# dsshim0125/s2p

Hardware: AMD Instinct MI355X
Metric: G+D train-step images/sec at 84x84 bs=64/GPU (higher is better)
Workload: dtype bf16; 1 GPU; configs[2]: full G+D train step (hinge GAN + feature matching + VGG19 perceptual + L1, Adam x2), 84x84 cheetah, netG=s2p, netD=multiscale(2); global_batch=64, per_gpu_batch=64, parallelism=dp1, hip_graph=True, graph_segments=1, streams=overlapped, vgg_weights=seeded stand-in (ImageNet weights unobtainable offline)

## Files before the change

### include/s2p_hip.h

```cpp
#ifndef S2P_HIP_H
#define S2P_HIP_H
#include <stddef.h>
#include <stdint.h>

#ifdef __cplusplus
extern "C" {
#endif
#pragma GCC visibility push(default)

#define S2P_VERSION 125

enum { S2P_F32 = 0, S2P_BF16 = 1 };
enum { S2P_ACT_NONE = 0, S2P_ACT_RELU = 1, S2P_ACT_LRELU = 2, S2P_ACT_TANH = 3, S2P_ACT_SWISH = 4 };
enum { S2P_EPI_STORE = 0,
       S2P_EPI_ADD = 1,
       S2P_EPI_MUL_ACTGRAD = 2   };

typedef struct {
  int32_t dtype;
  int32_t N, H, W, Cin, x_pitch;
  int32_t Ho, Wo, Cout, y_pitch;
  int32_t KH, KW, stride, pad;
  int32_t transposed;
  int32_t reflect;
// ... 24 lines not shown
                       size_t workspace_bytes, void* stream);
int s2p_conv2d_dgrad_mat(const s2p_conv_desc* d, const void* dy, const void* w_bwd, void* d_mid, const void* aux, const void* xn,
                         int xn_pitch, const float* stats, const void* gb_img, int gb_pitch, const float* gb_st,
                         int gb_st_pitch, int act, float slope, float eps, float* sums, void* dxn, int dxn_pitch,
                         void* dgb_img, int dgb_pitch, float* dgb_st, int dgb_st_pitch, const void* res, int res_pitch,
                         void* workspace, size_t workspace_bytes, void* stream);
int s2p_conv2d_mat_is_fused(const s2p_conv_desc* d, int dgrad, int has_gb);
enum { S2P_CONV_PATH_THIN = 0, S2P_CONV_PATH_THIN4 = 1, S2P_CONV_PATH_THIN_CIN = 2, S2P_CONV_PATH_THIN_ROWS = 3,
       S2P_CONV_PATH_PLANE = 4, S2P_CONV_PATH_PLANEG = 5, S2P_CONV_PATH_HALO = 6, S2P_CONV_PATH_SPLITK = 7,
       S2P_CONV_PATH_DMA = 8, S2P_CONV_PATH_PHASES = 9, S2P_CONV_PATH_GENERIC = 10 };
enum { S2P_HALO_S9_176_PIPE = 0, S2P_HALO_S9_176 = 1, S2P_HALO_S9_320 = 2, S2P_HALO_R_176 = 3, S2P_HALO_R_320 = 4 };
int s2p_conv2d_path(const s2p_conv_desc* d, int dgrad, int has_workspace);
int s2p_conv2d_wgrad(const s2p_conv_desc* d, const void* x, const void* dy, float* dw, float* db,
                     int cin_real, int cout_real, int64_t dw_gstride, int splitk, void* stream);
size_t s2p_conv2d_wgrad_workspace(const s2p_conv_desc* d, int cin_real, int cout_real);
int s2p_conv2d_wgrad_ws(const s2p_conv_desc* d, const void* x, const void* dy, float* dw, float* db,
                        int cin_real, int cout_real, int64_t dw_gstride, int splitk, void* workspace,
                        size_t workspace_bytes, void* stream);
size_t s2p_conv2d_wgrad_det_workspace(const s2p_conv_desc* d, int cin_real, int cout_real, int splitk);
typedef struct { const void* x; const void* dy; float* dw; float* db; } s2p_wgrad_job;
size_t s2p_conv2d_wgrad_batched_workspace(const s2p_conv_desc* d, int n_jobs, int cin_real, int cout_real);
int s2p_conv2d_wgrad_batched(const s2p_conv_desc* d, const s2p_wgrad_job* jobs, int n_jobs, int cin_real,
                             int cout_real, void* workspace, size_t workspace_bytes, void* stream);
int s2p_reflect_pad_bwd(int dtype, const void* dxp, int N, int H, int W, int C, int pad, void* dx,
                        void* stream);
int s2p_channel_sum(int dtype, const void* dy, int64_t pixels, int C, int pitch, float* db,
                    void* stream);
size_t s2p_channel_sum_workspace(int64_t pixels, int C);
int s2p_channel_sum_ws(int dtype, const void* dy, int64_t pixels, int C, int pitch, float* db, void* workspace,
                       size_t workspace_bytes, void* stream);

int64_t s2p_in_stats_floats(int N, int HW, int C);
int s2p_in_stats(int dtype, const void* x, int N, int HW, int C, int pitch, float eps,
                 float* stats, void* stream);
int s2p_in_apply_fwd(int dtype, const void* x, int N, int HW, int C, int pitch,
                     const float* stats, const void* gb_img, int gb_pitch,
                     const float* gb_st, int gb_st_pitch, int act, float slope, float eps,
                     void* y, int y_pitch, void* stream);
int s2p_in_norm_fwd(int dtype, const void* x, int N, int HW, int C, int pitch, const void* gb_img, int gb_pitch,
                    const float* gb_st, int gb_st_pitch, int act, float slope, float eps, void* y, int y_pitch,
                    float* stats, void* stream);
int64_t s2p_in_bwd_sums_floats(int N, int HW, int C);
int s2p_in_bwd_reduce(int dtype, const void* da, int da_pitch, const void* x, int N, int HW, int C,
                      int pitch, const float* stats, const void* gb_img, int gb_pitch,
                      const float* gb_st, int gb_st_pitch, int act, float slope, float eps,
                      float* sums, void* stream);
// ... 184 lines not shown
```

### s2p_amd/_lib.py

```python
import ctypes
import os
import subprocess

import torch

_HERE = os.path.dirname(os.path.abspath(__file__))
_SO = os.path.join(_HERE, "csrc", "libs2p_hip.so")

F32, BF16 = 0, 1
ACT_NONE, ACT_RELU, ACT_LRELU, ACT_TANH, ACT_SWISH = 0, 1, 2, 3, 4
EPI_STORE, EPI_ADD, EPI_MUL_ACTGRAD = 0, 1, 2
(PATH_THIN, PATH_THIN4, PATH_THIN_CIN, PATH_THIN_ROWS, PATH_PLANE, PATH_PLANEG, PATH_HALO, PATH_SPLITK, PATH_DMA, PATH_PHASES,
 PATH_GENERIC) = range(11)
HALO_S9_176_PIPE, HALO_S9_176, HALO_S9_320, HALO_R_176, HALO_R_320 = range(5)

c_int, c_float, c_void_p, c_int64 = ctypes.c_int, ctypes.c_float, ctypes.c_void_p, ctypes.c_int64


class ConvDesc(ctypes.Structure):
    _fields_ = [(n, ctypes.c_int32) for n in (
        "dtype", "N", "H", "W", "Cin", "x_pitch", "Ho", "Wo", "Cout", "y_pitch",
        "KH", "KW", "stride", "pad", "transposed", "reflect", "groups", "x_gstride", "y_gstride", "cin_real")]


# ... 34 lines not shown
SIGNATURES = {
    "s2p_version": [],
    "s2p_last_error": [],
    "s2p_conv2d_fwd": [_DESC, _P, _P, _P, _P, _P, c_int, c_float, c_int, _P],
    "s2p_conv2d_dgrad": [_DESC, _P, _P, _P, _P, _P, c_int, c_int, c_float, _P],
    "s2p_conv2d_fwd_workspace": [_DESC, c_int],
    "s2p_conv2d_fwd_ws": [_DESC, _P, _P, _P, _P, _P, c_int, c_float, c_int, _P, ctypes.c_size_t, _P],
    "s2p_conv2d_fwd_mat": [_DESC, _P, _P, _P, _P, _P, c_int, _P, c_int, _P, c_int, c_int, c_float, c_float, _P, c_int, _P, _P,
                           ctypes.c_size_t, _P],
    "s2p_conv2d_dgrad_mat": [_DESC, _P, _P, _P, _P, _P, c_int, _P, _P, c_int, _P, c_int, c_int, c_float, c_float, _P, _P, c_int, _P, c_int,
                             _P, c_int, _P, c_int, _P, ctypes.c_size_t, _P],
    "s2p_conv2d_mat_is_fused": [_DESC, c_int, c_int],
    "s2p_conv2d_path": [_DESC, c_int, c_int],
    "s2p_conv2d_dgrad_workspace": [_DESC],
    "s2p_conv2d_dgrad_ws": [_DESC, _P, _P, _P, _P, _P, c_int, c_int, c_float, _P, ctypes.c_size_t, _P],
    "s2p_conv2d_wgrad": [_DESC, _P, _P, _P, _P, c_int, c_int, c_int64, c_int, _P],
    "s2p_conv2d_wgrad_workspace": [_DESC, c_int, c_int],
    "s2p_conv2d_wgrad_det_workspace": [_DESC, c_int, c_int, c_int],
    "s2p_channel_sum_workspace": [c_int64, c_int],
    "s2p_channel_sum_ws": [c_int, _P, c_int64, c_int, c_int, _P, _P, ctypes.c_size_t, _P],
    "s2p_conv2d_wgrad_ws": [_DESC, _P, _P, _P, _P, c_int, c_int, c_int64, c_int, _P, ctypes.c_size_t, _P],
    "s2p_conv2d_wgrad_batched_workspace": [_DESC, c_int, c_int, c_int],
    "s2p_conv2d_wgrad_batched": [_DESC, ctypes.POINTER(WgradJob), c_int, c_int, c_int, _P, ctypes.c_size_t, _P],
    "s2p_reflect_pad_bwd": [c_int, _P, c_int, c_int, c_int, c_int, c_int, _P, _P],
    "s2p_channel_sum": [c_int, _P, c_int64, c_int, c_int, _P, _P],
    "s2p_in_stats": [c_int, _P, c_int, c_int, c_int, c_int, c_float, _P, _P],
    "s2p_in_apply_fwd": [c_int, _P, c_int, c_int, c_int, c_int, _P, _P, c_int, _P, c_int, c_int, c_float,
                         c_float, _P, c_int, _P],
    "s2p_in_norm_fwd": [c_int, _P, c_int, c_int, c_int, c_int, _P, c_int, _P, c_int, c_int, c_float, c_float, _P, c_int,
                        _P, _P],
    "s2p_in_bwd_reduce": [c_int, _P, c_int, _P, c_int, c_int, c_int, c_int, _P, _P, c_int, _P, c_int, c_int,
                          c_float, c_float, _P, _P],
    "s2p_in_bwd_apply": [c_int, _P, c_int, _P, c_int, c_int, c_int, c_int, _P, _P, c_int, _P, c_int, c_int,
                         c_float, c_float, _P, _P, c_int, _P, c_int, _P, c_int, _P],
    "s2p_in_norm_bwd": [c_int, _P, c_int, _P, c_int, c_int, c_int, c_int, _P, _P, c_int, _P, c_int, c_int,
                        c_float, c_float, _P, _P, c_int, _P, c_int, _P, c_int, _P],
    "s2p_in_norm_bwd_res": [c_int, _P, c_int, _P, c_int, c_int, c_int, c_int, _P, _P, c_int, _P, c_int, c_int,
                            c_float, c_float, _P, _P, c_int, _P, c_int, _P, c_int, _P, c_int, _P],
    "s2p_in_stats_floats": [c_int, c_int, c_int],
    "s2p_in_bwd_sums_floats": [c_int, c_int, c_int],
    "s2p_linear_fwd": [_P, c_int, c_int, c_int, _P, c_int, _P, c_int, c_int, c_float, _P, c_int, c_int, _P],
    "s2p_linear_bwd_workspace": [c_int, c_int, c_int],
    "s2p_linear_bwd": [_P, c_int, _P, c_int, _P, c_int, c_int, c_int, c_int, c_int, _P, c_int, c_int, c_float, _P, c_int, _P, _P,
                       c_int, _P, ctypes.c_size_t, _P],
    "s2p_gauss_head_fwd": [_P, c_int, c_int, c_int, _P, c_int, _P, c_int, _P, c_int, _P, c_int, _P, c_int, _P],
    "s2p_gauss_head_bwd": [_P, c_int, c_int, c_int, _P, c_int, _P, c_int, _P, c_int, _P, c_int, _P, c_int, _P, c_int, _P],
# ... 130 lines not shown
```

### s2p_amd/csrc/wgrad_slab.hip

```cpp
#include "wgrad_slab_core.h"

constexpr int WS_MAX_JOBS = 16;
struct WgSlabArgs {
  const void* A[WS_MAX_JOBS]; const void* B[WS_MAX_JOBS]; float* dW[WS_MAX_JOBS]; float* db[WS_MAX_JOBS];
  float* slab; float* slabb;
  WgsRaster g;
  int Cin;
  int co_tiles, tiles_per_job;
  int S, blocks_per_split, nblocks;
  int halo;
  int toff[9];
  int total_wgs;
};

template <int WROWS, bool TBL>
__global__ __launch_bounds__(256, 2) void wgrad_slab_kernel(const WgSlabArgs a) {
  constexpr int T = 9, NXI = WROWS / 32;
  constexpr int TOFF = TBL ? WGS_TBL_BYTES : 0;
  __shared__ __attribute__((aligned(1024))) char lds_all[TOFF + WGS_NST * wgs_stage_bytes(NXI)];
  const int f = wgs_xcd_spread(blockIdx.x, a.total_wgs);
  const int per_job = a.tiles_per_job * a.S;
  const int job = f / per_job;
  const int rem = f - job * per_job;
  const int split = rem / a.tiles_per_job, tile = rem - split * a.tiles_per_job;
  const int co_t = tile % a.co_tiles, ci_s = tile / a.co_tiles;
  const int b0 = split * a.blocks_per_split;
  int b1 = b0 + a.blocks_per_split; if (b1 > a.nblocks) b1 = a.nblocks;
  const int nblk = b1 - b0;
  const int wave = __builtin_amdgcn_readfirstlane(threadIdx.x >> 6);
  const bool do_bias = a.db[job] != nullptr && ci_s == 0 && (wave & 1) == 0;
  const WgsRaster g = {a.g.N, a.g.Ha, a.g.Wa, a.g.Ha, a.g.Wa, a.g.Hp, a.g.Wp, 1, 0, 0, a.g.a_pitch, a.g.b_pitch, a.g.a_bytes, a.g.b_bytes};

  f32x16 acc[T];
  f32x16 accb;
  wgs_accumulate<T, NXI, TBL>(g, a.A[job], a.B[job], a.toff, a.halo, co_t, ci_s, b0, nblk, do_bias, lds_all + TOFF,
                              (unsigned*)lds_all, acc, accb);

  const int tile_g = job * a.tiles_per_job + tile;
  if (a.S == 1) {
    const int lane = threadIdx.x & 63, r = lane & 31, h = lane >> 5, wa = wave >> 1, wb = wave & 1;
    float* dW = a.dW[job];
    const int row_len = T * a.Cin;
#pragma unroll
    for (int t = 0; t < T; ++t)
#pragma unroll
      for (int e = 0; e < 16; ++e) {
        const int co = co_t * 64 + 32 * wa + (e & 3) + 8 * (e >> 2) + 4 * h;
        float* o = dW + (size_t)co * row_len + t * a.Cin + ci_s * 64 + 32 * wb + r;
        *o += acc[t][e];
      }
    if (do_bias && r == 0) {
      float* db = a.db[job];
#pragma unroll
      for (int e = 0; e < 16; ++e) db[co_t * 64 + 32 * wa + (e & 3) + 8 * (e >> 2) + 4 * h] += accb[e];
    }
  } else {
    wgs_store_slab<T>(a.slab + ((size_t)tile_g * a.S + split) * (64 * T * 64), a.slabb + ((size_t)tile_g * a.S + split) * 64, acc, accb, do_bias);
  }
}

__global__ __launch_bounds__(256) void wgrad_slab_reduce_kernel(const WgSlabArgs a) {
  constexpr int T = 9;
  const int tile_g = blockIdx.x / T, t = blockIdx.x - tile_g * T;
  const int job = tile_g / a.tiles_per_job, tile = tile_g - job * a.tiles_per_job;
  const int co_t = tile % a.co_tiles, ci_s = tile / a.co_tiles;
  const float* sl = a.slab + (size_t)tile_g * a.S * (64 * T * 64);
  float* dW = a.dW[job];
  const int row_len = T * a.Cin;
#pragma unroll
  for (int u = 0; u < 4; ++u) {
    const int i = threadIdx.x + 256 * u;
    const int qd = i & 15, row = i >> 4;
    const size_t so = ((size_t)(row * T + t) * 16 + qd) * 4;
    f32x4 s = *(const f32x4*)(sl + so);
    for (int k = 1; k < a.S; ++k) s += *(const f32x4*)(sl + (size_t)k * (64 * T * 64) + so);
    float* o = dW + (size_t)(co_t * 64 + row) * row_len + t * a.Cin + ci_s * 64 + qd * 4;
    *(f32x4*)o = *(const f32x4*)o + s;
  }
  if (t == 0 && a.db[job] != nullptr && ci_s == 0 && threadIdx.x < 64) {
    const float* sb = a.slabb + (size_t)tile_g * a.S * 64;
    float s = sb[threadIdx.x];
    for (int k = 1; k < a.S; ++k) s += sb[k * 64 + threadIdx.x];
// ... 72 lines not shown
  bool tbl;
  a.g = ws_raster(d); wgs_limits(a.g, tbl);
  const int Wp = a.g.Wp;
  a.Cin = d->Cin;
  a.co_tiles = d->Cout / 64; a.tiles_per_job = a.co_tiles * (d->Cin / 64);
  a.nblocks = cdiv((long long)d->N * a.g.Hp * Wp, 64);
  a.S = ws_splits(d, n_jobs);
  a.blocks_per_split = cdiv(a.nblocks, a.S);
  a.halo = Wp + 1;
  const int wrows = ws_window_rows(a.halo);
  for (int ky = 0; ky < 3; ++ky)
    for (int kx = 0; kx < 3; ++kx) a.toff[ky * 3 + kx] = (ky - 1) * Wp + (kx - 1);
  const int tiles = n_jobs * a.tiles_per_job;
  a.total_wgs = tiles * a.S;
  if (a.S > 1) {
    const size_t need = (size_t)tiles * a.S * (64 * 9 * 64 + 64) * sizeof(float);
    if (!workspace || workspace_bytes < need)
      S2P_FAIL(-1, "s2p_conv2d_wgrad_batched: workspace of %zu bytes needed (s2p_conv2d_wgrad_batched_workspace), got %zu", need, workspace_bytes);
    a.slab = (float*)workspace;
    a.slabb = a.slab + (size_t)tiles * a.S * (64 * 9 * 64);
  }
  hipStream_t st = (hipStream_t)stream;
  dim3 grid(a.total_wgs);
  if (wrows <= 128) { if (tbl) hipLaunchKernelGGL((wgrad_slab_kernel<128, true>), grid, dim3(256), 0, st, a); else hipLaunchKernelGGL((wgrad_slab_kernel<128, false>), grid, dim3(256), 0, st, a); }
  else if (wrows <= 192) { if (tbl) hipLaunchKernelGGL((wgrad_slab_kernel<192, true>), grid, dim3(256), 0, st, a); else hipLaunchKernelGGL((wgrad_slab_kernel<192, false>), grid, dim3(256), 0, st, a); }
  else { if (tbl) hipLaunchKernelGGL((wgrad_slab_kernel<256, true>), grid, dim3(256), 0, st, a); else hipLaunchKernelGGL((wgrad_slab_kernel<256, false>), grid, dim3(256), 0, st, a); }
  S2P_CHECK_LAUNCH("wgrad_slab_kernel");
  if (a.S > 1) {
    hipLaunchKernelGGL(wgrad_slab_reduce_kernel, dim3(tiles * 9), dim3(256), 0, st, a);
    S2P_CHECK_LAUNCH("wgrad_slab_reduce_kernel");
  }
  return 0;
}
```

### s2p_amd/csrc/wgrad_slab_core.h

```cpp
#pragma once
#include "s2p_common.h"

struct WgsRaster {
  int N, Ha, Wa, Hb, Wb, Hp, Wp, bs, py, px;
  int a_pitch, b_pitch;
  unsigned a_bytes, b_bytes;
};

constexpr int WGS_TBL_MAX = 768;
constexpr int WGS_TBL_BYTES = 2 * WGS_TBL_MAX * 4;
constexpr int WGS_NST = 3;
constexpr int wgs_stage_bytes(int nxi) { return (64 + nxi * 32) * 128; }

__device__ __forceinline__ int wgs_xcd_spread(int bid, int nw) {
  const int q8 = nw >> 3, r8 = nw & 7, xcd = bid & 7, k = bid >> 3;
  return (xcd < r8 ? xcd * (q8 + 1) : r8 * (q8 + 1) + (xcd - r8) * q8) + k;
}

template <int T, int NXI, bool TBL>
__device__ __forceinline__ void wgs_accumulate(const WgsRaster& g, const void* A, const void* B, const int* toff, const int halo,
                                               const int co_t, const int ci_s, const int b0, const int nblk, const bool do_bias,
                                               char* const smem, unsigned* const ptab, f32x16 (&acc)[T], f32x16& accb) {
  constexpr int RS = 128, NST = WGS_NST;
  constexpr int ASTG = 64 * RS;
  constexpr int STG = wgs_stage_bytes(NXI);
  constexpr int NDMA = 2 + NXI;
  const int tid = threadIdx.x, lane = tid & 63;
  const int wave = __builtin_amdgcn_readfirstlane(tid >> 6);

  const unsigned OOB = 0x80000000u;
  const i32x4 ar = s2p_make_rsrc(A, g.a_bytes);
  const i32x4 br = s2p_make_rsrc(B, g.b_bytes);
  const unsigned lds0 = __builtin_amdgcn_readfirstlane(s2p_lds_addr(smem));

  const int lrow = lane >> 3, pch = lane & 7;
  const int a_cbyte = (co_t * 64) * 2, b_cbyte = (ci_s * 64) * 2;
  int pn[NDMA], prr[NDMA], pc[NDMA];
  int cb[NDMA];
  unsigned q4[NDMA], noffc[NDMA], tv[NDMA];
  const int HpWp = g.Hp * g.Wp;
  if constexpr (TBL) {
    for (int q = tid; q < HpWp; q += 256) {
      const int r = q / g.Wp, c = q - r * g.Wp;
      ptab[q] = (c < g.Wa && r < g.Ha) ? (unsigned)(r * g.Wa + c) * (unsigned)(g.a_pitch * 2) : 0xc0000000u;
      const int sy = r * g.bs + g.py, sx = c * g.bs + g.px;
      ptab[WGS_TBL_MAX + q] = (sy < g.Hb && sx < g.Wb) ? (unsigned)(sy * g.Wb + sx) * (unsigned)(g.b_pitch * 2) : 0xc0000000u;
    }
    __syncthreads();
  }
#pragma unroll
  for (int i = 0; i < NDMA; ++i) {
    const int row = (4 * (i < 2 ? i : i - 2) + wave) * 8 + lrow;
    int pos = b0 * 64 + row - (i < 2 ? 0 : halo);
    int nadj = 0;
    if (pos < 0) { pos += g.Hp * g.Wp; nadj = -1; }
    cb[i] = (i < 2 ? a_cbyte : b_cbyte) + ((pch ^ (((row >> 1) & 1) << 2)) * 16);
    if constexpr (TBL) {
      const int n = pos / HpWp, q = pos - n * HpWp;
      q4[i] = (unsigned)q * 4u;
      noffc[i] = (unsigned)((n + nadj) * (i < 2 ? g.Ha * g.Wa * g.a_pitch * 2 : g.Hb * g.Wb * g.b_pitch * 2) + cb[i]);
      tv[i] = ptab[(i < 2 ? 0 : WGS_TBL_MAX) + q];
    } else {
      const int q1 = pos / g.Wp;
      pc[i] = pos - q1 * g.Wp;
      const int n = q1 / g.Hp;
      prr[i] = q1 - n * g.Hp;
      pn[i] = n + nadj;
    }
  }
  const int a_pitch2 = g.a_pitch * 2, b_pitch2 = g.b_pitch * 2;
  const int adv_q = 64 / g.Wp, adv_c = 64 - adv_q * g.Wp, adv_n = adv_q / g.Hp, adv_r = adv_q - adv_n * g.Hp;
  const int tadv_n = 64 / HpWp;
  const unsigned tadv_q4 = (unsigned)(64 - tadv_n * HpWp) * 4u, HpWp4 = (unsigned)HpWp * 4u;
  const unsigned img_a = (unsigned)(g.Ha * g.Wa) * (unsigned)a_pitch2, img_b = (unsigned)(g.Hb * g.Wb) * (unsigned)b_pitch2;
  auto issue_one = [&](auto ic, unsigned base) {
    constexpr int i = decltype(ic)::value;
    if constexpr (TBL) {
      const unsigned off = tv[i] + noffc[i];
      if (i < 2) s2p_dma16(ar, base + (4 * i + wave) * 1024, (int)off);
      else s2p_dma16(br, base + ASTG + (4 * (i - 2) + wave) * 1024, (int)off);
      const unsigned img = i < 2 ? img_a : img_b;
      const unsigned qa = q4[i] + tadv_q4;
      const bool wrap = qa >= HpWp4;
      q4[i] = wrap ? qa - HpWp4 : qa;
      noffc[i] += (unsigned)tadv_n * img + (wrap ? img : 0u);
      tv[i] = *(const unsigned*)((const char*)(ptab + (i < 2 ? 0 : WGS_TBL_MAX)) + q4[i]);
    } else {
      int off;
      if constexpr (i < 2) {
        const bool ok = pc[i] < g.Wa && prr[i] < g.Ha && (unsigned)pn[i] < (unsigned)g.N;
        const int pix = __mul24(__mul24(pn[i], g.Ha) + prr[i], g.Wa) + pc[i];
        off = ok ? __mul24(pix, a_pitch2) + cb[i] : (int)OOB;
        s2p_dma16(ar, base + (4 * i + wave) * 1024, off);
      } else {
        const int sy = prr[i] * g.bs + g.py, sx = pc[i] * g.bs + g.px;
        const bool ok = sy < g.Hb && sx < g.Wb && (unsigned)pn[i] < (unsigned)g.N;
        const int pix = __mul24(__mul24(pn[i], g.Hb) + sy, g.Wb) + sx;
        off = ok ? __mul24(pix, b_pitch2) + cb[i] : (int)OOB;
        s2p_dma16(br, base + ASTG + (4 * (i - 2) + wave) * 1024, off);
      }
      int c = pc[i] + adv_c, r = prr[i] + adv_r, n = pn[i] + adv_n;
      const bool cw = c >= g.Wp;
      c = cw ? c - g.Wp : c; r += cw ? 1 : 0;
      const bool rw = r >= g.Hp;
      r = rw ? r - g.Hp : r; n += rw ? 1 : 0;
      pc[i] = c; prr[i] = r; pn[i] = n;
    }
  };
  auto issue = [&](int stage) {
    const unsigned base = lds0 + stage * STG;
    s2p_static_for<0, NDMA>([&](auto ic) { issue_one(ic, base); });
  };

  const int gq = lane >> 4, gg = gq & 1, hh = gq >> 1, q = (lane >> 2) & 3, p = lane & 3;
  const int wa = wave >> 1, wb = wave & 1;
  const int a_lane = (8 * hh + q) * RS + (((4 * wa + 2 * gg + (p >> 1)) ^ ((q >> 1) << 2)) * 16) + 8 * (p & 1);
  int b_lane[T];
#pragma unroll
  for (int t = 0; t < T; ++t) {
    const int r0 = halo + toff[t] + 8 * hh + q;
    b_lane[t] = ASTG + r0 * RS + (((4 * wb + 2 * gg + (p >> 1)) ^ (((r0 >> 1) & 1) << 2)) * 16) + 8 * (p & 1);
  }

#pragma unroll
  for (int e = 0; e < 16; ++e) accb[e] = 0.f;
#pragma unroll
  for (int t = 0; t < T; ++t)
#pragma unroll
    for (int e = 0; e < 16; ++e) acc[t][e] = 0.f;
  typedef __attribute__((ext_vector_type(8))) short s16x8;
  const s16x8 ones_s = {0x3f80, 0x3f80, 0x3f80, 0x3f80, 0x3f80, 0x3f80, 0x3f80, 0x3f80};
  const bf16x8 ones = __builtin_bit_cast(bf16x8, ones_s);
  typedef __attribute__((address_space(3))) s16x4* lds_s16x4;

  issue(0);
  if (nblk > 1) { issue(1); S2P_WAIT_VMCNT(NDMA); } else { S2P_WAIT_VMCNT(0); }
  __builtin_amdgcn_s_barrier();
  __builtin_amdgcn_sched_barrier(0);
  constexpr int NSTEP = 4 * T;
  constexpr int LA = NSTEP < 4 ? NSTEP : 4, RING = LA + 1;
  constexpr int TA = T - 1 - LA >= 0 ? T - 1 - LA : 0;
  auto read_frag = [&](const char* ptr) {
    s16x4 lo = __builtin_amdgcn_ds_read_tr16_b64_v4i16((lds_s16x4)(ptr));
    s16x4 hi = __builtin_amdgcn_ds_read_tr16_b64_v4i16((lds_s16x4)(ptr + 4 * RS));
    return __builtin_bit_cast(bf16x8, __builtin_shufflevector(lo, hi, 0, 1, 2, 3, 4, 5, 6, 7));
  };
  auto main_loop = [&](auto biasc) {
    constexpr bool BIAS = decltype(biasc)::value;
    int stage = 0;
    for (int kb = 0; kb < nblk; ++kb) {
      int st2 = stage + 2; if (st2 >= NST) st2 -= NST;
      const bool more = kb + 2 < nblk;
      const unsigned dbase = lds0 + st2 * STG;
      const char* sb = smem + stage * STG;
      bf16x8 AF[2], BF[RING];
      AF[0] = read_frag(sb + a_lane);
      s2p_static_for<0, LA>([&](auto vc) {
        constexpr int v = decltype(vc)::value;
        BF[v % RING] = read_frag(sb + b_lane[v % T] + (v / T) * 16 * RS);
      });
      s2p_static_for<0, NSTEP>([&](auto uc) {
        constexpr int u = decltype(uc)::value, s_ = u / T, t = u % T;
        if constexpr (BIAS && t == 0) accb = __builtin_amdgcn_mfma_f32_32x32x16_bf16(AF[s_ & 1], ones, accb, 0, 0, 0);
        acc[t] = __builtin_amdgcn_mfma_f32_32x32x16_bf16(AF[s_ & 1], BF[u % RING], acc[t], 0, 0, 0);
        constexpr int v = u + LA;
        if constexpr (v < NSTEP) BF[v % RING] = read_frag(sb + b_lane[v % T] + (v / T) * 16 * RS);
        if constexpr (t == TA && s_ < 3) AF[(s_ + 1) & 1] = read_frag(sb + a_lane + (s_ + 1) * 16 * RS);
        s2p_static_for<0, NDMA>([&](auto ic) {
          constexpr int i = decltype(ic)::value;
          constexpr int at = (i * NSTEP) / NDMA + 1 < NSTEP ? (i * NSTEP) / NDMA + 1 : NSTEP - 1;
          if constexpr (u == at) { if (more) issue_one(ic, dbase); }
        });
        __builtin_amdgcn_sched_barrier(0);
      });
      if (more) S2P_WAIT_VMCNT(NDMA); else S2P_WAIT_VMCNT(0);
      asm volatile("s_waitcnt lgkmcnt(0)" ::: "memory");
      __builtin_amdgcn_s_barrier();
      __builtin_amdgcn_sched_barrier(0);
      if (++stage == NST) stage = 0;
    }
  };
  if (do_bias) main_loop(std::integral_constant<bool, true>{});
  else main_loop(std::integral_constant<bool, false>{});
}

template <int T>
__device__ __forceinline__ void wgs_store_slab(float* sl, float* slb, const f32x16 (&acc)[T], const f32x16& accb, const bool do_bias) {
  const int lane = threadIdx.x & 63, wave = __builtin_amdgcn_readfirstlane(threadIdx.x >> 6);
  const int wa = wave >> 1, wb = wave & 1, r = lane & 31, h = lane >> 5;
#pragma unroll
  for (int t = 0; t < T; ++t)
#pragma unroll
    for (int e = 0; e < 16; ++e) {
      const int row = 32 * wa + (e & 3) + 8 * (e >> 2) + 4 * h;
      sl[(row * T + t) * 64 + 32 * wb + r] = acc[t][e];
    }
  if (do_bias && r == 0) {
#pragma unroll
    for (int e = 0; e < 16; ++e) slb[32 * wa + (e & 3) + 8 * (e >> 2) + 4 * h] = accb[e];
  }
}

static inline bool wgs_limits(WgsRaster& g, bool& tbl) {
  if ((long long)g.N * g.Hp * g.Wp >= (1 << 23) || (long long)g.N * g.Hb * g.Wb >= (1 << 23) || (long long)g.N * g.Ha * g.Wa >= (1 << 23)) return false;
  const long long ab = (long long)g.N * g.Ha * g.Wa * g.a_pitch * 2, bb = (long long)g.N * g.Hb * g.Wb * g.b_pitch * 2;
  if (ab >= (1ll << 31) || bb >= (1ll << 31)) return false;
  g.a_bytes = (unsigned)ab; g.b_bytes = (unsigned)bb;
  tbl = g.Hp * g.Wp <= WGS_TBL_MAX && ab <= (1ll << 29) && bb <= (1ll << 29) && !S2P_DIAG_SWITCH(18);
  return true;
}
```

### s2p_amd/csrc/wgrad_slabg.hip

```cpp
#include "wgrad_slab_core.h"

constexpr int SG_MAX_CLS = 4, SG_MAX_T = 8;
struct WgSlabGArgs {
  const void* A; const void* B; float* dW; float* db;
  float* slab; float* slabb;
  WgsRaster g;
  int co_tiles, tiles_per_cls;
  int dw_row, Cb;
  int ncls;
  int cls_T[SG_MAX_CLS], cls_py[SG_MAX_CLS], cls_px[SG_MAX_CLS], cls_hneg[SG_MAX_CLS];
  int cls_S[SG_MAX_CLS], cls_bps[SG_MAX_CLS];
  int cls_wg0[SG_MAX_CLS + 1];
  int cls_red0[SG_MAX_CLS + 1];
  long long cls_slab0[SG_MAX_CLS];
  int toff[SG_MAX_CLS][SG_MAX_T];
  int wt[SG_MAX_CLS][SG_MAX_T];
  int nblocks, total_wgs;
  int tbl;
};

template <int T, int NXI, bool TBL>
__device__ __forceinline__ void sg_body(const WgSlabGArgs& a, char* lds_all, const int cls, const int tile, const int split) {
  const int wave = __builtin_amdgcn_readfirstlane(threadIdx.x >> 6);
  const int co_t = tile % a.co_tiles, ci_s = tile / a.co_tiles;
  const int bps = a.cls_bps[cls];
  const int b0 = split * bps;
  int b1 = b0 + bps; if (b1 > a.nblocks) b1 = a.nblocks;
  const int nblk = b1 - b0;
  const bool do_bias = a.db != nullptr && cls == 0 && ci_s == 0 && (wave & 1) == 0;
  WgsRaster g = a.g;
  g.py = a.cls_py[cls]; g.px = a.cls_px[cls];

  f32x16 acc[T];
  f32x16 accb;
  wgs_accumulate<T, NXI, TBL>(g, a.A, a.B, a.toff[cls], a.cls_hneg[cls], co_t, ci_s, b0, nblk, do_bias,
                              lds_all + WGS_TBL_BYTES, (unsigned*)lds_all, acc, accb);

  const int S = a.cls_S[cls];
  wgs_store_slab<T>(a.slab + a.cls_slab0[cls] + ((size_t)tile * S + split) * (64 * T * 64), a.slabb + ((size_t)co_t * S + split) * 64,
                    acc, accb, do_bias);
}

template <int NXI>
__global__ __launch_bounds__(256, 2) void wgrad_slabg_kernel(const WgSlabGArgs a) {
  __shared__ __attribute__((aligned(1024))) char lds_all[WGS_TBL_BYTES + WGS_NST * wgs_stage_bytes(NXI)];
  const int f = wgs_xcd_spread(blockIdx.x, a.total_wgs);
  int cls = 0;
#pragma unroll
  for (int c = 1; c < SG_MAX_CLS; ++c) cls += (c < a.ncls && f >= a.cls_wg0[c]) ? 1 : 0;
  cls = __builtin_amdgcn_readfirstlane(cls);
  const int rem = f - a.cls_wg0[cls];
  const int split = rem / a.tiles_per_cls, tile = rem - split * a.tiles_per_cls;
  const int T = a.cls_T[cls];
  if (a.tbl) {
    if (T == 8) sg_body<8, NXI, true>(a, lds_all, cls, tile, split);
#ifdef S2P_DIAG_BUILD
    else if (T == 2) sg_body<2, NXI, true>(a, lds_all, cls, tile, split);
    else if (T == 1) sg_body<1, NXI, true>(a, lds_all, cls, tile, split);
#endif
    else sg_body<4, NXI, true>(a, lds_all, cls, tile, split);
    return;
  }
  if (T == 8) sg_body<8, NXI, false>(a, lds_all, cls, tile, split);
#ifdef S2P_DIAG_BUILD
  else if (T == 2) sg_body<2, NXI, false>(a, lds_all, cls, tile, split);
  else if (T == 1) sg_body<1, NXI, false>(a, lds_all, cls, tile, split);
#endif
  else sg_body<4, NXI, false>(a, lds_all, cls, tile, split);
}

__global__ __launch_bounds__(256) void wgrad_slabg_reduce_kernel(const WgSlabGArgs a) {
  __shared__ f32x4 red[4][64];
  __shared__ float redb[4][64];
  const int blk = blockIdx.x >> 4, rq = blockIdx.x & 15;
  int cls = 0;
#pragma unroll
  for (int c = 1; c < SG_MAX_CLS; ++c) cls += (c < a.ncls && blk >= a.cls_red0[c]) ? 1 : 0;
  const int T = a.cls_T[cls], S = a.cls_S[cls];
  const int rem = blk - a.cls_red0[cls];
  const int tile = rem / T, t = rem - tile * T;
  const int co_t = tile % a.co_tiles, ci_s = tile / a.co_tiles;
  const size_t chunk = (size_t)64 * T * 64;
  const float* sl = a.slab + a.cls_slab0[cls] + (size_t)tile * S * chunk;
  const int seg = threadIdx.x >> 6, j = threadIdx.x & 63;
  const int per = (S + 3) >> 2, k0 = seg * per, k1 = k0 + per < S ? k0 + per : S;
  const int qd = j & 15, row = rq * 4 + (j >> 4);
  const size_t so = ((size_t)(row * T + t) * 16 + qd) * 4;
  f32x4 s = {0.f, 0.f, 0.f, 0.f};
  int k = k0;
  for (; k + 8 <= k1; k += 8) {
    f32x4 v[8];
// ... 30 lines not shown
  int Ca, Cb;
  WgsRaster& g = a.g;
  if (!d->transposed) { g.Ha = d->Ho; g.Wa = d->Wo; g.Hb = d->H; g.Wb = d->W; Ca = d->Cout; Cb = d->Cin; g.a_pitch = d->y_pitch; g.b_pitch = d->x_pitch; }
  else { g.Ha = d->H; g.Wa = d->W; g.Hb = d->Ho; g.Wb = d->Wo; Ca = d->Cin; Cb = d->Cout; g.a_pitch = d->x_pitch; g.b_pitch = d->y_pitch; }
  g.N = d->N; g.bs = s; a.Cb = Cb; a.dw_row = K * K * Cb;
  a.co_tiles = Ca / 64; a.tiles_per_cls = a.co_tiles * (Cb / 64);
  int ta[16], tb[16], tc[16];
  int amin = 0, amax = 0, bmin = 0, bmax = 0;
  for (int ky = 0; ky < K; ++ky)
    for (int kx = 0; kx < K; ++kx) {
      const int t = ky * K + kx, dy = ky - pad, dx = kx - pad;
      if (s == 2) {
        const int py = dy & 1, px = dx & 1;
        ta[t] = (dy - py) >> 1; tb[t] = (dx - px) >> 1; tc[t] = py * 2 + px;
      } else { ta[t] = dy; tb[t] = dx; tc[t] = ky >> 1; }
      amin = ta[t] < amin ? ta[t] : amin; amax = ta[t] > amax ? ta[t] : amax;
      bmin = tb[t] < bmin ? tb[t] : bmin; bmax = tb[t] > bmax ? tb[t] : bmax;
    }
  const int Hsub = s == 2 ? (g.Hb + 1) / 2 : g.Hb, Wsub = s == 2 ? (g.Wb + 1) / 2 : g.Wb;
  g.Hp = g.Ha + amax > Hsub - amin ? g.Ha + amax : Hsub - amin;
  g.Wp = g.Wa + bmax > Wsub - bmin ? g.Wa + bmax : Wsub - bmin;
  bool tbl;
  if (!wgs_limits(g, tbl)) return false;
  a.tbl = tbl ? 1 : 0;
  a.nblocks = cdiv((long long)g.N * g.Hp * g.Wp, 64);
  const int ncand = s == 2 ? 4 : 2;
  int order[4] = {0, 1, 2, 3}, cnt[4] = {0, 0, 0, 0};
  for (int t = 0; t < K * K; ++t) ++cnt[tc[t]];
  for (int i = 0; i < ncand; ++i)
    for (int j = i + 1; j < ncand; ++j)
      if (cnt[order[j]] > cnt[order[i]]) { int o = order[i]; order[i] = order[j]; order[j] = o; }
  a.ncls = 0;
  int span = 0;
  for (int i = 0; i < ncand; ++i) {
    const int c = order[i];
    if (!cnt[c]) continue;
    if (cnt[c] != 4 && cnt[c] != 8 && !(k3 && (cnt[c] == 1 || cnt[c] == 2))) return false;
    const int k = a.ncls++;
    a.cls_T[k] = cnt[c]; a.cls_py[k] = s == 2 ? c >> 1 : 0; a.cls_px[k] = s == 2 ? c & 1 : 0;
    int lo = 0, hi = 0, n = 0;
    for (int t = 0; t < K * K; ++t)
      if (tc[t] == c) {
        const int off = ta[t] * g.Wp + tb[t];
        a.toff[k][n] = off; a.wt[k][n] = t; ++n;
        lo = off < lo ? off : lo; hi = off > hi ? off : hi;
      }
    a.cls_hneg[k] = -lo;
// ... 54 lines not shown
```

Measured before the change: 8111 images/sec.

## Unroll pixel table per block in wgrad slab kernels with staged table reads

The LDS pixel-offset table is now unrolled over images, with each entry pre-adding the image base offset. The table state advances once per block with shared scalar-like bookkeeping instead of per-DMA lane state. Table reads are issued a couple of MFMA steps ahead of each DMA so the LDS read latency is hidden. This cuts per-lane address arithmetic and VGPRs in the wgrad slab kernels. In exchange the table uses more LDS, the old per-lane scheme is kept behind a diagnostic switch, and a host helper for checking offsets is added.

```diff
diff --git a/include/s2p_hip.h b/include/s2p_hip.h
--- a/include/s2p_hip.h
+++ b/include/s2p_hip.h
@@ -70,6 +70,8 @@
 size_t s2p_conv2d_wgrad_batched_workspace(const s2p_conv_desc* d, int n_jobs, int cin_real, int cout_real);
 int s2p_conv2d_wgrad_batched(const s2p_conv_desc* d, const s2p_wgrad_job* jobs, int n_jobs, int cin_real,
                              int cout_real, void* workspace, size_t workspace_bytes, void* stream);
+int s2p_wgrad_slab_dma_offsets(const int* geom, int operand, int halo, int window_rows, int channel_tile, int first_block,
+                               int block, uint32_t* offsets, uint32_t* range_bytes);
 int s2p_reflect_pad_bwd(int dtype, const void* dxp, int N, int H, int W, int C, int pad, void* dx,
                         void* stream);
 int s2p_channel_sum(int dtype, const void* dy, int64_t pixels, int C, int pitch, float* db,
diff --git a/s2p_amd/_lib.py b/s2p_amd/_lib.py
--- a/s2p_amd/_lib.py
+++ b/s2p_amd/_lib.py
@@ -80,6 +80,7 @@
     "s2p_conv2d_wgrad_ws": [_DESC, _P, _P, _P, _P, c_int, c_int, c_int64, c_int, _P, ctypes.c_size_t, _P],
     "s2p_conv2d_wgrad_batched_workspace": [_DESC, c_int, c_int, c_int],
     "s2p_conv2d_wgrad_batched": [_DESC, ctypes.POINTER(WgradJob), c_int, c_int, c_int, _P, ctypes.c_size_t, _P],
+    "s2p_wgrad_slab_dma_offsets": [_P, c_int, c_int, c_int, c_int, c_int, c_int, _P, _P],
     "s2p_reflect_pad_bwd": [c_int, _P, c_int, c_int, c_int, c_int, c_int, _P, _P],
     "s2p_channel_sum": [c_int, _P, c_int64, c_int, c_int, _P, _P],
     "s2p_in_stats": [c_int, _P, c_int, c_int, c_int, c_int, c_float, _P, _P],
diff --git a/s2p_amd/csrc/wgrad_slab.hip b/s2p_amd/csrc/wgrad_slab.hip
--- a/s2p_amd/csrc/wgrad_slab.hip
+++ b/s2p_amd/csrc/wgrad_slab.hip
@@ -13,10 +13,10 @@
   int total_wgs;
 };
 
-template <int WROWS, bool TBL>
-__global__ __launch_bounds__(256, 2) void wgrad_slab_kernel(const WgSlabArgs a) {
+template <int WROWS, int MODE>
+__device__ __forceinline__ void ws_body(const WgSlabArgs& a) {
   constexpr int T = 9, NXI = WROWS / 32;
-  constexpr int TOFF = TBL ? WGS_TBL_BYTES : 0;
+  constexpr int TOFF = MODE != WGS_NRC ? wgs_tbl_bytes(NXI) : 0;
   __shared__ __attribute__((aligned(1024))) char lds_all[TOFF + WGS_NST * wgs_stage_bytes(NXI)];
   const int f = wgs_xcd_spread(blockIdx.x, a.total_wgs);
   const int per_job = a.tiles_per_job * a.S;
@@ -33,8 +33,8 @@
 
   f32x16 acc[T];
   f32x16 accb;
-  wgs_accumulate<T, NXI, TBL>(g, a.A[job], a.B[job], a.toff, a.halo, co_t, ci_s, b0, nblk, do_bias, lds_all + TOFF,
-                              (unsigned*)lds_all, acc, accb);
+  wgs_accumulate<T, NXI, MODE>(g, a.A[job], a.B[job], a.toff, a.halo, co_t, ci_s, b0, nblk, do_bias, lds_all + TOFF,
+                               (unsigned*)lds_all, acc, accb);
 
   const int tile_g = job * a.tiles_per_job + tile;
   if (a.S == 1) {
@@ -58,6 +58,13 @@
     wgs_store_slab<T>(a.slab + ((size_t)tile_g * a.S + split) * (64 * T * 64), a.slabb + ((size_t)tile_g * a.S + split) * 64, acc, accb, do_bias);
   }
 }
+
+template <int WROWS, bool TBL>
+__global__ __launch_bounds__(256, 2) void wgrad_slab_kernel(const WgSlabArgs a) { ws_body<WROWS, TBL ? WGS_TBL : WGS_NRC>(a); }
+#ifdef S2P_DIAG_BUILD
+template <int WROWS>
+__global__ __launch_bounds__(256, 2) void wgrad_slab_lane_kernel(const WgSlabArgs a) { ws_body<WROWS, WGS_TBL_LANE>(a); }
+#endif
 
 __global__ __launch_bounds__(256) void wgrad_slab_reduce_kernel(const WgSlabArgs a) {
   constexpr int T = 9;
@@ -176,6 +183,13 @@
   }
   hipStream_t st = (hipStream_t)stream;
   dim3 grid(a.total_wgs);
+#ifdef S2P_DIAG_BUILD
+  if (tbl && S2P_DIAG_SWITCH(21)) {
+    if (wrows <= 128) hipLaunchKernelGGL((wgrad_slab_lane_kernel<128>), grid, dim3(256), 0, st, a);
+    else if (wrows <= 192) hipLaunchKernelGGL((wgrad_slab_lane_kernel<192>), grid, dim3(256), 0, st, a);
+    else hipLaunchKernelGGL((wgrad_slab_lane_kernel<256>), grid, dim3(256), 0, st, a);
+  } else
+#endif
   if (wrows <= 128) { if (tbl) hipLaunchKernelGGL((wgrad_slab_kernel<128, true>), grid, dim3(256), 0, st, a); else hipLaunchKernelGGL((wgrad_slab_kernel<128, false>), grid, dim3(256), 0, st, a); }
   else if (wrows <= 192) { if (tbl) hipLaunchKernelGGL((wgrad_slab_kernel<192, true>), grid, dim3(256), 0, st, a); else hipLaunchKernelGGL((wgrad_slab_kernel<192, false>), grid, dim3(256), 0, st, a); }
   else { if (tbl) hipLaunchKernelGGL((wgrad_slab_kernel<256, true>), grid, dim3(256), 0, st, a); else hipLaunchKernelGGL((wgrad_slab_kernel<256, false>), grid, dim3(256), 0, st, a); }
@@ -186,3 +200,36 @@
   }
   return 0;
 }
+
+extern "C" int s2p_wgrad_slab_dma_offsets(const int* geom, int operand, int halo, int window_rows, int channel_tile, int first_block,
+                                          int block, uint32_t* offsets, uint32_t* range_bytes) {
+  if (!geom || !offsets || !range_bytes || (operand != 0 && operand != 1)) S2P_FAIL(-1, "s2p_wgrad_slab_dma_offsets: bad argument");
+  WgsRaster g{};
+  g.N = geom[0]; g.Ha = geom[1]; g.Wa = geom[2]; g.Hb = geom[3]; g.Wb = geom[4]; g.Hp = geom[5]; g.Wp = geom[6];
+  g.bs = geom[7]; g.py = geom[8]; g.px = geom[9]; g.a_pitch = geom[10]; g.b_pitch = geom[11];
+  if (g.N < 1 || g.Ha < 1 || g.Wa < 1 || g.Hb < 1 || g.Wb < 1 || g.Hp < 1 || g.Wp < 1 || g.bs < 1 || g.a_pitch < 64 || g.b_pitch < 64)
+    S2P_FAIL(-1, "s2p_wgrad_slab_dma_offsets: bad geometry");
+  const int HpWp = g.Hp * g.Wp;
+  if (window_rows < 96 || window_rows > 256 || window_rows % 32 || halo < 0 || halo >= HpWp || channel_tile < 0 || first_block < 0 ||
+      block < first_block)
+    S2P_FAIL(-1, "s2p_wgrad_slab_dma_offsets: bad window / block");
+  bool tbl;
+  if (!wgs_limits(g, tbl)) S2P_FAIL(-2, "s2p_wgrad_slab_dma_offsets: beyond the kernels' addressing");
+  if (!tbl) return 0;
+  const int nxi = window_rows / 32, rows = operand == 0 ? 64 : window_rows;
+  unsigned ta[WGS_TBL_A], tb[WGS_TBL_MAX + 256];
+  wgs_tbl_fill(g, nxi, ta, tb, 0, 1);
+  const unsigned img = wgs_img_bytes(g, operand);
+  WgsTblBase s = wgs_tbl_base(first_block * 64 - (operand == 0 ? 0 : halo), HpWp, img);
+  const WgsTblStep st = wgs_tbl_step(HpWp);
+  for (int b = first_block; b < block; ++b) wgs_tbl_advance(s, st, img);
+  const unsigned* t = operand == 0 ? ta : tb;
+  for (int row = 0; row < rows; ++row)
+    for (int pch = 0; pch < 8; ++pch) {
+      const int lrow = row & 7;
+      const unsigned cb = (unsigned)(channel_tile * 128) + (unsigned)((pch ^ (((lrow >> 1) & 1) << 2)) * 16);
+      offsets[row * 8 + pch] = t[s.q4 / 4 + row] + cb + s.nim;
+    }
+  *range_bytes = operand == 0 ? g.a_bytes : g.b_bytes;
+  return rows;
+}
diff --git a/s2p_amd/csrc/wgrad_slab_core.h b/s2p_amd/csrc/wgrad_slab_core.h
--- a/s2p_amd/csrc/wgrad_slab_core.h
+++ b/s2p_amd/csrc/wgrad_slab_core.h
@@ -8,16 +8,56 @@
 };
 
 constexpr int WGS_TBL_MAX = 768;
-constexpr int WGS_TBL_BYTES = 2 * WGS_TBL_MAX * 4;
+constexpr unsigned WGS_TBL_PAD = 0xc0000000u;
+constexpr int WGS_TBL_A = WGS_TBL_MAX + 64;
+constexpr int wgs_tbl_bytes(int nxi) { return (WGS_TBL_A + WGS_TBL_MAX + nxi * 32) * 4; }
+enum { WGS_NRC = 0, WGS_TBL = 1, WGS_TBL_LANE = 2 };
 constexpr int WGS_NST = 3;
 constexpr int wgs_stage_bytes(int nxi) { return (64 + nxi * 32) * 128; }
+
+__host__ __device__ inline unsigned wgs_tbl_pixel(const WgsRaster& g, const int op, const int r, const int c) {
+  if (op == 0) return (c < g.Wa && r < g.Ha) ? (unsigned)(r * g.Wa + c) * (unsigned)(g.a_pitch * 2) : WGS_TBL_PAD;
+  const int sy = r * g.bs + g.py, sx = c * g.bs + g.px;
+  return (sy < g.Hb && sx < g.Wb) ? (unsigned)(sy * g.Wb + sx) * (unsigned)(g.b_pitch * 2) : WGS_TBL_PAD;
+}
+__host__ __device__ inline unsigned wgs_img_bytes(const WgsRaster& g, const int op) {
+  return op == 0 ? (unsigned)(g.Ha * g.Wa) * (unsigned)(g.a_pitch * 2) : (unsigned)(g.Hb * g.Wb) * (unsigned)(g.b_pitch * 2);
+}
+__host__ __device__ inline void wgs_tbl_fill(const WgsRaster& g, const int nxi, unsigned* ta, unsigned* tb, const int tid, const int nthr) {
+  const int HpWp = g.Hp * g.Wp;
+  const unsigned img_a = wgs_img_bytes(g, 0), img_b = wgs_img_bytes(g, 1);
+  for (int q = tid; q < HpWp; q += nthr) {
+    const int r = q / g.Wp, c = q - r * g.Wp;
+    unsigned e = wgs_tbl_pixel(g, 0, r, c);
+    for (int x = q; x < HpWp + 64; x += HpWp, e += img_a) ta[x] = e;
+    e = wgs_tbl_pixel(g, 1, r, c);
+    for (int x = q; x < HpWp + nxi * 32; x += HpWp, e += img_b) tb[x] = e;
+  }
+}
+struct WgsTblBase { unsigned q4, nim; };
+struct WgsTblStep { unsigned aq4, H4; int an; };
+__host__ __device__ inline WgsTblStep wgs_tbl_step(const int HpWp) {
+  const int an = 64 / HpWp;
+  return {(unsigned)(64 - an * HpWp) * 4u, (unsigned)HpWp * 4u, an};
+}
+__host__ __device__ inline WgsTblBase wgs_tbl_base(const int pos, const int HpWp, const unsigned img) {
+  const int p = pos + HpWp, n = p / HpWp;
+  return {(unsigned)(p - n * HpWp) * 4u, (unsigned)(n - 1) * img};
+}
+__host__ __device__ inline void wgs_tbl_advance(WgsTblBase& s, const WgsTblStep& st, const unsigned img) {
+  const unsigned q = s.q4 + st.aq4;
+  const bool wrap = q >= st.H4;
+  s.q4 = wrap ? q - st.H4 : q;
+  s.nim += (unsigned)st.an * img + (wrap ? img : 0u);
+}
+constexpr int wgs_dma_step(int i, int nstep, int ndma) { return (i * nstep) / ndma + 1 < nstep ? (i * nstep) / ndma + 1 : nstep - 1; }
 
 __device__ __forceinline__ int wgs_xcd_spread(int bid, int nw) {
   const int q8 = nw >> 3, r8 = nw & 7, xcd = bid & 7, k = bid >> 3;
   return (xcd < r8 ? xcd * (q8 + 1) : r8 * (q8 + 1) + (xcd - r8) * q8) + k;
 }
 
-template <int T, int NXI, bool TBL>
+template <int T, int NXI, int MODE>
 __device__ __forceinline__ void wgs_accumulate(const WgsRaster& g, const void* A, const void* B, const int* toff, const int halo,
                                                const int co_t, const int ci_s, const int b0, const int nblk, const bool do_bias,
                                                char* const smem, unsigned* const ptab, f32x16 (&acc)[T], f32x16& accb) {
@@ -33,33 +73,49 @@
   const i32x4 br = s2p_make_rsrc(B, g.b_bytes);
   const unsigned lds0 = __builtin_amdgcn_readfirstlane(s2p_lds_addr(smem));
 
+  constexpr bool TBL = MODE == WGS_TBL, LANE = MODE == WGS_TBL_LANE;
   const int lrow = lane >> 3, pch = lane & 7;
   const int a_cbyte = (co_t * 64) * 2, b_cbyte = (ci_s * 64) * 2;
   int pn[NDMA], prr[NDMA], pc[NDMA];
   int cb[NDMA];
   unsigned q4[NDMA], noffc[NDMA], tv[NDMA];
   const int HpWp = g.Hp * g.Wp;
+  const unsigned img_a = wgs_img_bytes(g, 0), img_b = wgs_img_bytes(g, 1);
+  constexpr int LANE_B = WGS_TBL_MAX;
+  const unsigned swz = (unsigned)((pch ^ (((lrow >> 1) & 1) << 2)) * 16);
+  const unsigned cba = (unsigned)a_cbyte + swz, cbb = (unsigned)b_cbyte + swz;
+  const unsigned lane4 = (unsigned)(wave * 8 + lrow) * 4u;
+  WgsTblBase tsa{}, tsb{};
+  const WgsTblStep tstep = wgs_tbl_step(HpWp);
+  unsigned nim_a = 0, nim_b = 0, tva = 0, tvb = 0;
   if constexpr (TBL) {
+    wgs_tbl_fill(g, NXI, ptab, ptab + WGS_TBL_A, tid, 256);
+    tsa = wgs_tbl_base(b0 * 64, HpWp, img_a);
+    tsb = wgs_tbl_base(b0 * 64 - halo, HpWp, img_b);
+    __syncthreads();
+  }
+#ifdef S2P_DIAG_BUILD
+  if constexpr (LANE) {
     for (int q = tid; q < HpWp; q += 256) {
       const int r = q / g.Wp, c = q - r * g.Wp;
-      ptab[q] = (c < g.Wa && r < g.Ha) ? (unsigned)(r * g.Wa + c) * (unsigned)(g.a_pitch * 2) : 0xc0000000u;
-      const int sy = r * g.bs + g.py, sx = c * g.bs + g.px;
-      ptab[WGS_TBL_MAX + q] = (sy < g.Hb && sx < g.Wb) ? (unsigned)(sy * g.Wb + sx) * (unsigned)(g.b_pitch * 2) : 0xc0000000u;
+      ptab[q] = wgs_tbl_pixel(g, 0, r, c);
+      ptab[LANE_B + q] = wgs_tbl_pixel(g, 1, r, c);
     }
     __syncthreads();
   }
-#pragma unroll
-  for (int i = 0; i < NDMA; ++i) {
+#endif
+#pragma unroll
+  for (int i = 0; i < (TBL ? 0 : NDMA); ++i) {
     const int row = (4 * (i < 2 ? i : i - 2) + wave) * 8 + lrow;
     int pos = b0 * 64 + row - (i < 2 ? 0 : halo);
     int nadj = 0;
     if (pos < 0) { pos += g.Hp * g.Wp; nadj = -1; }
     cb[i] = (i < 2 ? a_cbyte : b_cbyte) + ((pch ^ (((row >> 1) & 1) << 2)) * 16);
-    if constexpr (TBL) {
+    if constexpr (LANE) {
       const int n = pos / HpWp, q = pos - n * HpWp;
       q4[i] = (unsigned)q * 4u;
       noffc[i] = (unsigned)((n + nadj) * (i < 2 ? g.Ha * g.Wa * g.a_pitch * 2 : g.Hb * g.Wb * g.b_pitch * 2) + cb[i]);
-      tv[i] = ptab[(i < 2 ? 0 : WGS_TBL_MAX) + q];
+      tv[i] = ptab[(i < 2 ? 0 : LANE_B) + q];
     } else {
       const int q1 = pos / g.Wp;
       pc[i] = pos - q1 * g.Wp;
@@ -70,12 +126,25 @@
   }
   const int a_pitch2 = g.a_pitch * 2, b_pitch2 = g.b_pitch * 2;
   const int adv_q = 64 / g.Wp, adv_c = 64 - adv_q * g.Wp, adv_n = adv_q / g.Hp, adv_r = adv_q - adv_n * g.Hp;
-  const int tadv_n = 64 / HpWp;
-  const unsigned tadv_q4 = (unsigned)(64 - tadv_n * HpWp) * 4u, HpWp4 = (unsigned)HpWp * 4u;
-  const unsigned img_a = (unsigned)(g.Ha * g.Wa) * (unsigned)a_pitch2, img_b = (unsigned)(g.Hb * g.Wb) * (unsigned)b_pitch2;
+  auto tbl_next_block = [&]() {
+    tva = lane4 + tsa.q4; tvb = lane4 + tsb.q4;
+    nim_a = tsa.nim; nim_b = tsb.nim;
+    wgs_tbl_advance(tsa, tstep, img_a);
+    wgs_tbl_advance(tsb, tstep, img_b);
+  };
+  auto tbl_read = [&](auto ic) {
+    constexpr int i = decltype(ic)::value;
+    if constexpr (i < 2) tv[i] = *(const unsigned*)((const char*)ptab + tva + i * 128);
+    else tv[i] = *(const unsigned*)((const char*)ptab + tvb + (WGS_TBL_A * 4 + (i - 2) * 128));
+  };
   auto issue_one = [&](auto ic, unsigned base) {
     constexpr int i = decltype(ic)::value;
     if constexpr (TBL) {
+      if (i < 2) s2p_dma16(ar, base + (4 * i + wave) * 1024, (int)(tv[i] + cba + nim_a));
+      else s2p_dma16(br, base + ASTG + (4 * (i - 2) + wave) * 1024, (int)(tv[i] + cbb + nim_b));
+#ifdef S2P_DIAG_BUILD
+    } else if constexpr (LANE) {
+      const unsigned tadv_q4 = tstep.aq4, HpWp4 = tstep.H4;
       const unsigned off = tv[i] + noffc[i];
       if (i < 2) s2p_dma16(ar, base + (4 * i + wave) * 1024, (int)off);
       else s2p_dma16(br, base + ASTG + (4 * (i - 2) + wave) * 1024, (int)off);
@@ -83,8 +152,9 @@
       const unsigned qa = q4[i] + tadv_q4;
       const bool wrap = qa >= HpWp4;
       q4[i] = wrap ? qa - HpWp4 : qa;
-      noffc[i] += (unsigned)tadv_n * img + (wrap ? img : 0u);
-      tv[i] = *(const unsigned*)((const char*)(ptab + (i < 2 ? 0 : WGS_TBL_MAX)) + q4[i]);
+      noffc[i] += (unsigned)tstep.an * img + (wrap ? img : 0u);
+      tv[i] = *(const unsigned*)((const char*)(ptab + (i < 2 ? 0 : LANE_B)) + q4[i]);
+#endif
     } else {
       int off;
       if constexpr (i < 2) {
@@ -109,6 +179,10 @@
   };
   auto issue = [&](int stage) {
     const unsigned base = lds0 + stage * STG;
+    if constexpr (TBL) {
+      tbl_next_block();
+      s2p_static_for<0, NDMA>([&](auto ic) { tbl_read(ic); });
+    }
     s2p_static_for<0, NDMA>([&](auto ic) { issue_one(ic, base); });
   };
 
@@ -140,6 +214,7 @@
   constexpr int NSTEP = 4 * T;
   constexpr int LA = NSTEP < 4 ? NSTEP : 4, RING = LA + 1;
   constexpr int TA = T - 1 - LA >= 0 ? T - 1 - LA : 0;
+  constexpr int TLA = 2;
   auto read_frag = [&](const char* ptr) {
     s16x4 lo = __builtin_amdgcn_ds_read_tr16_b64_v4i16((lds_s16x4)(ptr));
     s16x4 hi = __builtin_amdgcn_ds_read_tr16_b64_v4i16((lds_s16x4)(ptr + 4 * RS));
@@ -154,6 +229,10 @@
       const unsigned dbase = lds0 + st2 * STG;
       const char* sb = smem + stage * STG;
       bf16x8 AF[2], BF[RING];
+      if constexpr (TBL) {
+        tbl_next_block();
+        s2p_static_for<0, NDMA>([&](auto ic) { if constexpr (wgs_dma_step(decltype(ic)::value, NSTEP, NDMA) - TLA < 0) tbl_read(ic); });
+      }
       AF[0] = read_frag(sb + a_lane);
       s2p_static_for<0, LA>([&](auto vc) {
         constexpr int v = decltype(vc)::value;
@@ -168,7 +247,8 @@
         if constexpr (t == TA && s_ < 3) AF[(s_ + 1) & 1] = read_frag(sb + a_lane + (s_ + 1) * 16 * RS);
         s2p_static_for<0, NDMA>([&](auto ic) {
           constexpr int i = decltype(ic)::value;
-          constexpr int at = (i * NSTEP) / NDMA + 1 < NSTEP ? (i * NSTEP) / NDMA + 1 : NSTEP - 1;
+          constexpr int at = wgs_dma_step(i, NSTEP, NDMA);
+          if constexpr (TBL && u == at - TLA) tbl_read(ic);
           if constexpr (u == at) { if (more) issue_one(ic, dbase); }
         });
         __builtin_amdgcn_sched_barrier(0);
@@ -206,6 +286,7 @@
   const long long ab = (long long)g.N * g.Ha * g.Wa * g.a_pitch * 2, bb = (long long)g.N * g.Hb * g.Wb * g.b_pitch * 2;
   if (ab >= (1ll << 31) || bb >= (1ll << 31)) return false;
   g.a_bytes = (unsigned)ab; g.b_bytes = (unsigned)bb;
-  tbl = g.Hp * g.Wp <= WGS_TBL_MAX && ab <= (1ll << 29) && bb <= (1ll << 29) && !S2P_DIAG_SWITCH(18);
+  tbl = g.Hp * g.Wp <= WGS_TBL_MAX && ab <= (1ll << 29) && bb <= (1ll << 29) && g.a_pitch <= (1 << 15) && g.b_pitch <= (1 << 15) &&
+        !S2P_DIAG_SWITCH(18);
   return true;
 }
diff --git a/s2p_amd/csrc/wgrad_slabg.hip b/s2p_amd/csrc/wgrad_slabg.hip
--- a/s2p_amd/csrc/wgrad_slabg.hip
+++ b/s2p_amd/csrc/wgrad_slabg.hip
@@ -19,7 +19,7 @@
   int tbl;
 };
 
-template <int T, int NXI, bool TBL>
+template <int T, int NXI, int MODE>
 __device__ __forceinline__ void sg_body(const WgSlabGArgs& a, char* lds_all, const int cls, const int tile, const int split) {
   const int wave = __builtin_amdgcn_readfirstlane(threadIdx.x >> 6);
   const int co_t = tile % a.co_tiles, ci_s = tile / a.co_tiles;
@@ -33,8 +33,8 @@
 
   f32x16 acc[T];
   f32x16 accb;
-  wgs_accumulate<T, NXI, TBL>(g, a.A, a.B, a.toff[cls], a.cls_hneg[cls], co_t, ci_s, b0, nblk, do_bias,
-                              lds_all + WGS_TBL_BYTES, (unsigned*)lds_all, acc, accb);
+  wgs_accumulate<T, NXI, MODE>(g, a.A, a.B, a.toff[cls], a.cls_hneg[cls], co_t, ci_s, b0, nblk, do_bias,
+                               lds_all + wgs_tbl_bytes(NXI), (unsigned*)lds_all, acc, accb);
 
   const int S = a.cls_S[cls];
   wgs_store_slab<T>(a.slab + a.cls_slab0[cls] + ((size_t)tile * S + split) * (64 * T * 64), a.slabb + ((size_t)co_t * S + split) * 64,
@@ -43,7 +43,7 @@
 
 template <int NXI>
 __global__ __launch_bounds__(256, 2) void wgrad_slabg_kernel(const WgSlabGArgs a) {
-  __shared__ __attribute__((aligned(1024))) char lds_all[WGS_TBL_BYTES + WGS_NST * wgs_stage_bytes(NXI)];
+  __shared__ __attribute__((aligned(1024))) char lds_all[wgs_tbl_bytes(NXI) + WGS_NST * wgs_stage_bytes(NXI)];
   const int f = wgs_xcd_spread(blockIdx.x, a.total_wgs);
   int cls = 0;
 #pragma unroll
@@ -52,21 +52,30 @@
   const int rem = f - a.cls_wg0[cls];
   const int split = rem / a.tiles_per_cls, tile = rem - split * a.tiles_per_cls;
   const int T = a.cls_T[cls];
+#ifdef S2P_DIAG_BUILD
+  if (a.tbl == WGS_TBL_LANE) {
+    if (T == 8) sg_body<8, NXI, WGS_TBL_LANE>(a, lds_all, cls, tile, split);
+    else if (T == 2) sg_body<2, NXI, WGS_TBL_LANE>(a, lds_all, cls, tile, split);
+    else if (T == 1) sg_body<1, NXI, WGS_TBL_LANE>(a, lds_all, cls, tile, split);
+    else sg_body<4, NXI, WGS_TBL_LANE>(a, lds_all, cls, tile, split);
+    return;
+  }
+#endif
   if (a.tbl) {
-    if (T == 8) sg_body<8, NXI, true>(a, lds_all, cls, tile, split);
+    if (T == 8) sg_body<8, NXI, WGS_TBL>(a, lds_all, cls, tile, split);
 #ifdef S2P_DIAG_BUILD
-    else if (T == 2) sg_body<2, NXI, true>(a, lds_all, cls, tile, split);
-    else if (T == 1) sg_body<1, NXI, true>(a, lds_all, cls, tile, split);
+    else if (T == 2) sg_body<2, NXI, WGS_TBL>(a, lds_all, cls, tile, split);
+    else if (T == 1) sg_body<1, NXI, WGS_TBL>(a, lds_all, cls, tile, split);
 #endif
-    else sg_body<4, NXI, true>(a, lds_all, cls, tile, split);
+    else sg_body<4, NXI, WGS_TBL>(a, lds_all, cls, tile, split);
     return;
   }
-  if (T == 8) sg_body<8, NXI, false>(a, lds_all, cls, tile, split);
+  if (T == 8) sg_body<8, NXI, WGS_NRC>(a, lds_all, cls, tile, split);
 #ifdef S2P_DIAG_BUILD
-  else if (T == 2) sg_body<2, NXI, false>(a, lds_all, cls, tile, split);
-  else if (T == 1) sg_body<1, NXI, false>(a, lds_all, cls, tile, split);
+  else if (T == 2) sg_body<2, NXI, WGS_NRC>(a, lds_all, cls, tile, split);
+  else if (T == 1) sg_body<1, NXI, WGS_NRC>(a, lds_all, cls, tile, split);
 #endif
-  else sg_body<4, NXI, false>(a, lds_all, cls, tile, split);
+  else sg_body<4, NXI, WGS_NRC>(a, lds_all, cls, tile, split);
 }
 
 __global__ __launch_bounds__(256) void wgrad_slabg_reduce_kernel(const WgSlabGArgs a) {
@@ -143,7 +152,7 @@
   g.Wp = g.Wa + bmax > Wsub - bmin ? g.Wa + bmax : Wsub - bmin;
   bool tbl;
   if (!wgs_limits(g, tbl)) return false;
-  a.tbl = tbl ? 1 : 0;
+  a.tbl = tbl ? (S2P_DIAG_SWITCH(21) ? WGS_TBL_LANE : WGS_TBL) : WGS_NRC;
   a.nblocks = cdiv((long long)g.N * g.Hp * g.Wp, 64);
   const int ncand = s == 2 ? 4 : 2;
   int order[4] = {0, 1, 2, 3}, cnt[4] = {0, 0, 0, 0};
```

Result: no change. 8133 images/sec, median of 6 (+0.3%).
